# usnistgov/alignn

Hardware: NVIDIA B200
Metric: graphs/sec fwd+bwd (higher is better)
Workload: dtype f32

## Files before the change

### alignn_b200/_lib.py

```python
from __future__ import annotations

import ctypes as C
import os
from typing import Optional

import torch

_HERE = os.path.dirname(os.path.abspath(__file__))
LIB_PATH = os.path.join(_HERE, "libalignn_b200.so")

NORM_LAYER, NORM_AFFINE, NORM_STATS = 0, 1, 2
SUPPORTED_D = (32, 64, 128, 256)

_fp = C.c_void_p


class EgcFwdArgs(C.Structure):
    _fields_ = [
        ("struct_size", C.c_size_t),
        ("Nn", C.c_int64), ("Ne", C.c_int64),
        ("d", C.c_int32), ("norm_nodes", C.c_int32), ("norm_edges", C.c_int32), ("residual", C.c_int32),
        ("gate_is_m", C.c_int32),
        ("gate_eps", C.c_float), ("ln_eps", C.c_float),
        ("x", _fp), ("y", _fp), ("G", _fp), ("P", _fp),
        ("src", _fp), ("in_ptr", _fp), ("in_eid", _fp),
        ("n_w", _fp), ("n_b", _fp), ("e_w", _fp), ("e_b", _fp),
        ("x_out", _fp), ("y_out", _fp), ("M", _fp), ("XP", _fp), ("S", _fp), ("H", _fp),
        ("partials", _fp),
        ("stream", _fp),
    ]


class EgcBwdArgs(C.Structure):
    _fields_ = [
        ("struct_size", C.c_size_t),
        ("Nn", C.c_int64), ("Ne", C.c_int64),
        ("d", C.c_int32), ("norm_nodes", C.c_int32), ("norm_edges", C.c_int32),
        ("gate_eps", C.c_float), ("ln_eps", C.c_float),
        ("P", _fp), ("M", _fp), ("XP", _fp), ("S", _fp), ("H", _fp),
        ("src", _fp), ("dst", _fp), ("in_ptr", _fp), ("in_eid", _fp), ("out_ptr", _fp), ("out_eid", _fp),
        ("n_w", _fp), ("n_b", _fp), ("n_mean", _fp), ("n_rstd", _fp),
        ("e_w", _fp), ("e_b", _fp), ("e_mean", _fp), ("e_rstd", _fp),
        ("n_c1", _fp), ("n_c2", _fp), ("e_c1", _fp), ("e_c2", _fp),
        ("gx_out", _fp), ("gy_out", _fp),
        ("GM", _fp), ("GP", _fp), ("GSh", _fp),
        ("partials", _fp), ("partials_src", _fp),
        ("stream", _fp),
    ]


class GemmGatherArgs(C.Structure):
    _fields_ = [
        ("struct_size", C.c_size_t),
        ("M", C.c_int64), ("N", C.c_int32), ("K", C.c_int32),
        ("A", _fp), ("lda", C.c_int64),
        ("w_image", _fp), ("bias", _fp),
        ("add0", _fp), ("ld0", C.c_int64), ("idx0", _fp),
        ("add1", _fp), ("ld1", C.c_int64), ("idx1", _fp),
        ("C", _fp), ("ldc", C.c_int64),
        ("stats", _fp),
        ("bn_scale", _fp), ("bn_shift", _fp), ("bn_mean", _fp),
        ("stream", _fp),
    ]


class WgradProblem(C.Structure):
    _fields_ = [("A", _fp), ("lda", C.c_int64), ("B", _fp), ("ldb", C.c_int64), ("K", C.c_int64), ("out", _fp), ("ld_out", C.c_int64)]


class ColsumProblem(C.Structure):
    _fields_ = [("a", _fp), ("rows", C.c_int64), ("stride", C.c_int64), ("cols", C.c_int), ("alpha", C.c_float), ("out", _fp)]


class ImageEntry(C.Structure):
    _fields_ = [("W", _fp), ("ldw", C.c_int64), ("rows", C.c_int32), ("cols", C.c_int32), ("transpose", C.c_int32),
                ("n_off", C.c_int32), ("k_off", C.c_int32), ("N", C.c_int32), ("K", C.c_int32), ("image", _fp)]


class BiasEntry(C.Structure):
    _fields_ = [("a", _fp), ("b", _fp), ("dst", _fp), ("n", C.c_int32)]


_SIGNATURES = {
    "alignn_b200_version": (C.c_int, []),
    "alignn_b200_strerror": (C.c_char_p, [C.c_int]),
    "alignn_b200_last_cuda_error": (C.c_int, []),
    "alignn_b200_launch_count": (C.c_uint64, []),
    "alignn_b200_egc_partial_rows": (C.c_int, [C.c_int64, C.c_int]),
    "alignn_b200_egc_forward": (C.c_int, [C.POINTER(EgcFwdArgs)]),
    "alignn_b200_bn_finalize": (C.c_int, [_fp, C.c_int, C.c_int, C.c_int, C.c_int64, C.c_int, _fp, _fp, C.c_float,
                                          C.c_float, _fp, _fp, _fp, _fp, _fp, _fp, _fp]),
    "alignn_b200_affine_silu_residual": (C.c_int, [_fp, _fp, _fp, _fp, _fp, C.c_int64, C.c_int, _fp]),
    "alignn_b200_egc_backward": (C.c_int, [C.POINTER(EgcBwdArgs)]),
    "alignn_b200_bn_backward_reduce": (C.c_int, [_fp, _fp, _fp, _fp, _fp, _fp, C.c_int64, C.c_int, _fp, C.c_int, _fp]),
    "alignn_b200_rowstats_partials": (C.c_int, [_fp, C.c_int64, C.c_int, _fp, C.c_int, _fp]),
    "alignn_b200_bn_backward_apply": (C.c_int, [_fp, _fp, _fp, _fp, _fp, _fp, _fp, _fp, C.c_int64, C.c_int, _fp, _fp]),
    "alignn_b200_ln_silu_forward": (C.c_int, [_fp, _fp, _fp, C.c_float, C.c_int64, C.c_int, _fp, _fp, _fp]),
    "alignn_b200_ln_silu_backward": (C.c_int, [_fp, _fp, _fp, _fp, _fp, C.c_int64, C.c_int, _fp, _fp, C.c_int, _fp]),
    "alignn_b200_adamw_flat": (C.c_int, [_fp, _fp, _fp, _fp, C.c_int64, C.c_float, C.c_float, C.c_float, C.c_float, C.c_float,
                                         C.c_int, _fp, _fp, _fp]),
    "alignn_b200_colsum_partials": (C.c_int, [_fp, C.c_int64, C.c_int, _fp, C.c_int, _fp]),
    "alignn_b200_colsum": (C.c_int, [_fp, C.c_int64, C.c_int, C.c_int64, C.c_float, _fp, _fp]),
    "alignn_b200_colsum_batch": (C.c_int, [C.POINTER(ColsumProblem), C.c_int, _fp]),
    "alignn_b200_gather_segment_sum": (C.c_int, [_fp, _fp, _fp, _fp, _fp, C.c_int64, C.c_int64, C.c_int, _fp, _fp, _fp]),
    "alignn_b200_gemm_weight_image_bytes": (C.c_size_t, [C.c_int, C.c_int]),
    "alignn_b200_gemm_prepare_weights": (C.c_int, [_fp, C.c_int, C.c_int, C.c_int64, C.c_int, _fp, _fp]),
    "alignn_b200_gemm_prepare_table": (C.c_int, [_fp, C.c_int, C.c_int64, _fp, C.c_int, _fp]),
    "alignn_b200_gemm_nt": (C.c_int, [_fp, C.c_int64, _fp, C.c_int64, C.c_int, C.c_int, _fp, _fp, C.c_int64, _fp,
                                      C.c_int64, _fp]),
    "alignn_b200_gemm_gather": (C.c_int, [C.POINTER(GemmGatherArgs)]),
    "alignn_b200_gemm_gather_stat_rows": (C.c_int, [C.c_int64, C.c_int]),
    "alignn_b200_wgrad_workspace_bytes": (C.c_size_t, [C.c_int64, C.c_int, C.c_int, C.c_int]),
    "alignn_b200_wgrad_batch_workspace_bytes": (C.c_size_t, [C.POINTER(WgradProblem), C.c_int, C.c_int]),
    "alignn_b200_wgrad_batch": (C.c_int, [C.POINTER(WgradProblem), C.c_int, C.c_int, _fp, C.c_size_t, _fp]),
    "alignn_b200_wgrad": (C.c_int, [_fp, C.c_int64, _fp, C.c_int64, C.c_int64, C.c_int, C.c_int, C.c_int, _fp, C.c_int64,
                                    _fp, C.c_size_t, _fp]),
    "alignn_b200_csr_build_host": (C.c_int, [_fp, _fp, C.c_int64, C.c_int64, _fp, _fp, _fp, _fp, _fp, _fp, _fp, _fp]),
    "alignn_b200_line_graph_count_host": (C.c_int64, [_fp, _fp, _fp, C.c_int64]),
    "alignn_b200_line_graph_build_host": (C.c_int, [_fp, _fp, _fp, C.c_int64, _fp, C.c_int64, C.c_int64, _fp, _fp, _fp]),
    "alignn_b200_radius_graph_count_host": (C.c_int64, [_fp, _fp, C.c_int64, C.c_int64, C.c_double, C.c_double]),
    "alignn_b200_radius_graph_build_host": (C.c_int, [_fp, _fp, C.c_int64, C.c_int64, C.c_double, C.c_double, C.c_int64, _fp,
                                                      _fp, _fp, _fp]),
    "alignn_b200_csr_build_workspace_bytes": (C.c_size_t, [C.c_int64, C.c_int64]),
    "alignn_b200_csr_build": (C.c_int, [_fp, _fp, C.c_int64, C.c_int64, _fp, _fp, _fp, _fp, _fp, _fp, C.c_size_t, _fp]),
    "alignn_b200_line_graph_workspace_bytes": (C.c_size_t, [C.c_int64]),
    "alignn_b200_line_graph_offsets": (C.c_int, [_fp, _fp, _fp, C.c_int64, _fp, _fp, C.c_size_t, _fp]),
    "alignn_b200_line_graph_fill": (C.c_int, [_fp, _fp, _fp, _fp, C.c_int64, _fp, _fp, _fp, _fp]),
    "alignn_b200_radius_graph_workspace_bytes": (C.c_size_t, [C.c_int64]),
    "alignn_b200_radius_graph_offsets": (C.c_int, [_fp, _fp, C.c_int64, C.c_int64, C.c_double, C.c_double, _fp, _fp, C.c_size_t, _fp]),
    "alignn_b200_radius_graph_fill": (C.c_int, [_fp, _fp, C.c_int64, C.c_int64, C.c_double, C.c_double, _fp, _fp, _fp, _fp, _fp, _fp]),
    "alignn_b200_pair_force_scatter": (C.c_int, [_fp, _fp, _fp, _fp, _fp, C.c_int64, C.c_int, _fp, _fp]),
    "alignn_b200_virial_stress": (C.c_int, [_fp, _fp, _fp, _fp, _fp, C.c_int64, C.c_float, _fp, _fp]),
    "alignn_b200_debug_gemm_flags": (None, [C.c_int]),
    "alignn_b200_debug_gemm_pair": (None, [C.c_int]),
    "alignn_b200_debug_egc_flags": (None, [C.c_int]),
    "alignn_b200_debug_gemm_trace": (None, [_fp]),
    "alignn_b200_segment_mean": (C.c_int, [_fp, _fp, C.c_int64, C.c_int, _fp, _fp]),
    "alignn_b200_segment_mean_backward": (C.c_int, [_fp, _fp, C.c_int64, C.c_int, _fp, _fp]),
}

EXPORTED_SYMBOLS = tuple(_SIGNATURES)

_lib: Optional[C.CDLL] = None


def load() -> C.CDLL:
    global _lib
    if _lib is not None:
        return _lib
    if not os.path.exists(LIB_PATH):
        raise RuntimeError(
            f"{LIB_PATH} not found: the CUDA extension is not built. Run `python -c 'import __graft_entry__ as g; "
            "g.build()'` (nvcc, sm_100a). alignn_b200 has no CPU or eager fallback.")
    lib = C.CDLL(LIB_PATH)
    for name, (res, args) in _SIGNATURES.items():
        fn = getattr(lib, name)
        fn.restype, fn.argtypes = res, args
    if lib.alignn_b200_version() != 100:
        raise RuntimeError("libalignn_b200.so version mismatch; rebuild")
    _lib = lib
    return lib


def check(status: int, what: str) -> None:
    if status != 0:
        lib = load()
        msg = lib.alignn_b200_strerror(status).decode()
        extra = ""
        if status == -4:
            extra = f" (cudaError {lib.alignn_b200_last_cuda_error()})"
        raise RuntimeError(f"{what} failed: {msg}{extra}")


def launch_count() -> int:
    return int(load().alignn_b200_launch_count())


def ptr(t: Optional[torch.Tensor]):
    if t is None:
        return None
    return t.data_ptr()


def stream_ptr() -> int:
    return torch.cuda.current_stream().cuda_stream


def require_cuda(*tensors: torch.Tensor) -> None:
    for t in tensors:
        if t is None:
            continue
        if not t.is_cuda:
            raise RuntimeError("alignn_b200 kernels need CUDA tensors (no CPU path exists); got a tensor on "
                               f"{t.device}. Move the model and graphs to a B200 with .to('cuda').")
        if t.dtype not in (torch.float32, torch.int32):
            raise RuntimeError(f"alignn_b200 kernels are fp32/int32 only; got {t.dtype}")
        if not t.is_contiguous():
            raise RuntimeError("alignn_b200 kernels need contiguous tensors")
```

### alignn_b200/csrc/gemm_fused_tc.cu

```cuda
#include <atomic>
#include <cuda.h>

#include "tc_common.cuh"
#include "api_common.h"
#include "alignn_b200.h"

namespace alignn {
namespace gemm2 {

int make_map_f32(CUtensorMap* map, const float* base, int64_t rows, int64_t cols, int64_t ld, int box_rows);

constexpr int BM = 128;
constexpr int BK = 32;
constexpr int NSA = 3;
constexpr int NSP = 2;
constexpr int NSB = 3;
constexpr int EPI_WARPS = 8;
constexpr int CONV_WARPS = 4;
constexpr int THREADS = 32 * (4 + EPI_WARPS + CONV_WARPS);
constexpr uint32_t LBO = 128;
constexpr uint32_t SBO = (BK / 8) * 128;
constexpr int A_STAGE = BM * BK * 4;
constexpr int A_PLANE = BM * BK * 2;
constexpr int EPI_BOX = 32 * 32 * 4;
constexpr bool kTmaStore = true;
constexpr int EPI_BUFS = 1;

template <int BN>
struct Cfg {
  static constexpr int B_PLANE = BN * BK * 2;
  static constexpr int OFF_ASTG = 0;
  static constexpr int OFF_APL = OFF_ASTG + NSA * A_STAGE;
  static constexpr int OFF_B = OFF_APL + NSP * 2 * A_PLANE;
  static constexpr int OFF_EPI = (OFF_B + NSB * 2 * B_PLANE + 1023) / 1024 * 1024;
  static constexpr int EPI_BYTES = EPI_WARPS * EPI_BUFS * EPI_BOX;
  static constexpr int OFF_STAT = OFF_EPI + EPI_BYTES;
  static constexpr int STAT_BYTES = 4 * 2 * BN * 4;
  static constexpr int OFF_BAR = OFF_STAT + STAT_BYTES;
  static constexpr int SMEM = OFF_BAR + 256;
  static constexpr int TMEM_COLS = 2 * BN < 32 ? 32 : 2 * BN;
  static_assert(SMEM <= 232448, "shared memory budget of one sm_100 CTA");
};

struct Params {
  int M, N, K;
  const uint8_t* w_image;
  const float* bias;
  const float* add0; int64_t ld0; const int32_t* idx0;
  const float* add1; int64_t ld1; const int32_t* idx1;
  float* C; int64_t ldc;
  float* stats;
  int stat_quarters;
  const float* bn_scale; const float* bn_shift; const float* bn_mean;
  long long* trace;
};

#define GEMM2_TRACE(role, ctr) do { if (p.trace && blockIdx.x == 0 && (ctr) < 512) p.trace[(role) * 512 + (ctr)++] = clock64(); } while (0)

__host__ __device__ constexpr int plane_off(int r, int k) { return (r >> 3) * (int)SBO + (k >> 3) * 128 + (r & 7) * 16 + (k & 7) * 2; }

__device__ __forceinline__ float dsilu_(float u) {
  float e, sg;
  asm("ex2.approx.ftz.f32 %0, %1;" : "=f"(e) : "f"(u * -1.4426950408889634f));
  asm("rcp.approx.ftz.f32 %0, %1;" : "=f"(sg) : "f"(1.f + e));
  return sg * (1.f + u * (1.f - sg));
}
__device__ __forceinline__ void tma_load_2d(void* dst, const CUtensorMap* map, int c0, int c1, uint64_t* bar) {
  asm volatile("cp.async.bulk.tensor.2d.shared::cta.global.tile.mbarrier::complete_tx::bytes [%0], [%1, {%2, %3}], [%4];"
               ::"r"(tc::smem_u32(dst)), "l"(map), "r"(c0), "r"(c1), "r"(tc::smem_u32(bar)) : "memory");
}
__device__ __forceinline__ void tma_store_2d(const CUtensorMap* map, const void* src, int c0, int c1) {
  asm volatile("cp.async.bulk.tensor.2d.global.shared::cta.tile.bulk_group [%0, {%2, %3}], [%1];"
               ::"l"(map), "r"(tc::smem_u32(src)), "r"(c0), "r"(c1) : "memory");
}
__device__ __forceinline__ void tma_prefetch_2d(const CUtensorMap* map, int c0, int c1) {
  asm volatile("cp.async.bulk.prefetch.tensor.2d.L2.global.tile [%0, {%1, %2}];" ::"l"(map), "r"(c0), "r"(c1) : "memory");
}

template <int BN, int MODE>
__global__ void __launch_bounds__(THREADS, 1)
gemm_gather_bf16x3_kernel(const __grid_constant__ CUtensorMap mapA, const __grid_constant__ CUtensorMap mapC, const Params p) {
  using F = Cfg<BN>;
  extern __shared__ __align__(1024) uint8_t smem[];
  uint64_t* astg_full = reinterpret_cast<uint64_t*>(smem + F::OFF_BAR);
  uint64_t* astg_empty = astg_full + NSA;
  uint64_t* apl_full = astg_empty + NSA;
  uint64_t* apl_empty = apl_full + NSP;
  uint64_t* b_full = apl_empty + NSP;
  uint64_t* b_empty = b_full + NSB;
  uint64_t* tfull = b_empty + NSB;
  uint64_t* tempty = tfull + 2;
  uint32_t* tmem_slot = reinterpret_cast<uint32_t*>(tempty + 2);

  const int tid = threadIdx.x, warp = tid >> 5, lane = tid & 31;
  const int nk = p.K / BK;
  const int n_tiles = p.N / BN;
  const int m_tiles = (p.M + BM - 1) / BM;
  const int total = m_tiles * n_tiles;
  const int my_tiles = (total - (int)blockIdx.x + (int)gridDim.x - 1) / (int)gridDim.x;

  if (tid == 0) {
    for (int s = 0; s < NSA; ++s) { tc::mbar_init(&astg_full[s], 1); tc::mbar_init(&astg_empty[s], CONV_WARPS); }
    for (int s = 0; s < NSP; ++s) { tc::mbar_init(&apl_full[s], CONV_WARPS); tc::mbar_init(&apl_empty[s], 1); }
    for (int s = 0; s < NSB; ++s) { tc::mbar_init(&b_full[s], 1); tc::mbar_init(&b_empty[s], 1); }
    for (int a = 0; a < 2; ++a) { tc::mbar_init(&tfull[a], 1); tc::mbar_init(&tempty[a], EPI_WARPS); }
    tc::mbar_fence_init();
  }
  if (warp == 0) tc::tmem_alloc(tmem_slot, F::TMEM_COLS);
  tc::fence_before_sync();
  __syncthreads();
  tc::fence_after_sync();
  const uint32_t tmem = *tmem_slot;

  if (warp == 1) {
    if (lane == 0) {
      asm volatile("prefetch.tensormap [%0];" ::"l"(&mapA) : "memory");
      int c = 0, tr = 0;
      for (int lt = 0; lt < my_tiles; ++lt) {
        const int tile = blockIdx.x + lt * gridDim.x;
        const int m0 = (tile / n_tiles) * BM;
        if (lt + 1 < my_tiles) {
          const int nm0 = ((tile + (int)gridDim.x) / n_tiles) * BM;
          if (nm0 != m0)
            for (int kc = 0; kc < nk; ++kc) tma_prefetch_2d(&mapA, kc * BK, nm0);
        }
        for (int kc = 0; kc < nk; ++kc, ++c) {
          const int s = c % NSA;
          if (c >= NSA) tc::mbar_wait(&astg_empty[s], ((c / NSA) - 1) & 1);
          GEMM2_TRACE(0, tr);
          tc::mbar_arrive_expect_tx(&astg_full[s], A_STAGE);
          tma_load_2d(smem + F::OFF_ASTG + s * A_STAGE, &mapA, kc * BK, m0, &astg_full[s]);
        }
      }
    }
  } else if (warp == 2) {
    if (lane == 0) {
      int c = 0, trb = 0;
      for (int lt = 0; lt < my_tiles; ++lt) {
        const int tile = blockIdx.x + lt * gridDim.x;
        const uint8_t* wsrc = p.w_image + (int64_t)(tile % n_tiles) * nk * 2 * F::B_PLANE;
        for (int kc = 0; kc < nk; ++kc, ++c) {
          const int s = c % NSB;
          if (c >= NSB) tc::mbar_wait(&b_empty[s], ((c / NSB) - 1) & 1);
          GEMM2_TRACE(1, trb);
          tc::mbar_arrive_expect_tx(&b_full[s], 2 * F::B_PLANE);
          tc::bulk_g2s(smem + F::OFF_B + s * 2 * F::B_PLANE, wsrc, 2 * F::B_PLANE, &b_full[s]);
          wsrc += 2 * F::B_PLANE;
        }
      }
    }
  } else if (warp >= 4 + EPI_WARPS) {
    const int cw = warp - (4 + EPI_WARPS);
    int ld_off[8], st_off[8];
#pragma unroll
    for (int i = 0; i < 8; ++i) {
      const int u = (i * CONV_WARPS + cw) * 2 + (lane >> 4);
      const int row = (u >> 2) * 8 + (lane & 7);
      const int kq = (u & 3) * 2 + ((lane >> 3) & 1);
      ld_off[i] = row * 128 + ((kq ^ (row & 7)) << 4);
      st_off[i] = plane_off(row, kq * 4);
    }
    const int nchunks = my_tiles * nk;
    int tr2 = 0, tr3 = 0;
    for (int c = 0; c < nchunks; ++c) {
      const int sa = c % NSA, sp = c % NSP;
      tc::mbar_wait(&astg_full[sa], (c / NSA) & 1);
      if (cw == 0 && lane == 0) GEMM2_TRACE(2, tr2);
      const uint8_t* src = smem + F::OFF_ASTG + sa * A_STAGE;
      float4 v[8];
#pragma unroll
      for (int i = 0; i < 8; ++i) v[i] = *reinterpret_cast<const float4*>(src + ld_off[i]);
      if (c >= NSP) tc::mbar_wait(&apl_empty[sp], ((c / NSP) - 1) & 1);
      uint8_t* dst = smem + F::OFF_APL + sp * 2 * A_PLANE;
#pragma unroll
      for (int i = 0; i < 8; ++i) {
        uint2 hi, lo;
        tc::split4(v[i], hi, lo);
        *reinterpret_cast<uint2*>(dst + st_off[i]) = hi;
        *reinterpret_cast<uint2*>(dst + A_PLANE + st_off[i]) = lo;
      }
      tc::fence_async_smem();
      __syncwarp();
      if (lane == 0) {
        tc::mbar_arrive(&apl_full[sp]);
        tc::mbar_arrive(&astg_empty[sa]);
      }
      if (cw == 0 && lane == 0) GEMM2_TRACE(3, tr3);
    }
  } else if (warp >= 4) {
    const int ew = warp - 4;
    const int q = warp & 3;
    uint8_t* stg0 = smem + F::OFF_EPI + ew * EPI_BUFS * EPI_BOX;
    const int st_row = lane * 128, st_sw = lane & 7;
    uint32_t chunk_ctr = 0;
    float* stat = reinterpret_cast<float*>(smem + F::OFF_STAT) + q * 2 * BN;
    const int half = ew >> 2;
    constexpr bool bnmode = MODE == 1;
    constexpr bool plain = MODE == 2 && kTmaStore;
    constexpr bool one = MODE == 3;
    constexpr bool late_wait = (plain || one) && kTmaStore;
    const bool do_stats = !plain && !one && p.stats != nullptr;
    if (do_stats)
      for (int ch = half; ch < BN / 32; ch += 2) { stat[ch * 32 + lane] = 0.f; stat[BN + ch * 32 + lane] = 0.f; }
    const int rsub = lane >> 3;
    const int c4 = (lane & 7) * 4;
    constexpr int NCH = BN / 32;
    uint32_t lt = 0;
    int tr5 = 0;
    for (int tile = blockIdx.x; tile < total; tile += gridDim.x, ++lt) {
      const int acc = lt & 1;
      const int m0 = (tile / n_tiles) * BM, n0 = (tile % n_tiles) * BN;
      int i0[8], i1[8];
      uint32_t rvm = 0;
      const float* base0 = p.add0 + n0 + c4 + half * 32;
      const float* base1 = p.add1 + n0 + c4 + half * 32;
      float4 a0[8], a1[8];
      const float4 z4 = make_float4(0.f, 0.f, 0.f, 0.f);
      if constexpr (!plain) {
#pragma unroll
        for (int it = 0; it < 8; ++it) {
          const int gr = m0 + q * 32 + it * 4 + rsub;
          const bool ok = gr < p.M;
          rvm |= (ok ? 1u : 0u) << it;
          i0[it] = (p.add0 && ok) ? (p.idx0 ? __ldg(p.idx0 + gr) : gr) : -1;
          if constexpr (!one) i1[it] = (p.add1 && ok) ? (p.idx1 ? __ldg(p.idx1 + gr) : gr) : -1;
        }
#pragma unroll
        for (int it = 0; it < 8; ++it) {
          a0[it] = (i0[it] >= 0 && half < NCH) ? __ldg(reinterpret_cast<const float4*>(base0 + (int64_t)i0[it] * p.ld0)) : z4;
          if constexpr (!one)
            a1[it] = (i1[it] >= 0 && half < NCH) ? __ldg(reinterpret_cast<const float4*>(base1 + (int64_t)i1[it] * p.ld1)) : z4;
        }
      }
      tc::mbar_wait(&tfull[acc], (lt >> 1) & 1);
      tc::fence_after_sync();
      if (ew == 0 && lane == 0) GEMM2_TRACE(5, tr5);
#pragma unroll 1
      for (int ch = half; ch < NCH; ch += 2) {
        const int c0 = ch * 32;
        uint8_t* stg = stg0;
        if (!late_wait && kTmaStore && chunk_ctr >= 1) {
          if (lane == 0) asm volatile("cp.async.bulk.wait_group.read 0;" ::: "memory");
          __syncwarp();
        }
        {
          float v[32];
          tc::tmem_ld32(tmem + ((uint32_t)(q * 32) << 16) + (uint32_t)(acc * BN + c0), v);
          if (ew == 0 && lane == 0) GEMM2_TRACE(5, tr5);
          if (late_wait && chunk_ctr >= 1) {
            if (lane == 0) asm volatile("cp.async.bulk.wait_group.read 0;" ::: "memory");
            __syncwarp();
          }
          ++chunk_ctr;
          if constexpr (plain) {
            if (p.bias) {
#pragma unroll
              for (int j = 0; j < 8; ++j) {
                const float4 b = __ldg(reinterpret_cast<const float4*>(p.bias + n0 + c0 + 4 * j));
                v[4 * j] += b.x; v[4 * j + 1] += b.y; v[4 * j + 2] += b.z; v[4 * j + 3] += b.w;
              }
            }
          }
#pragma unroll
          for (int j = 0; j < 8; ++j)
            *reinterpret_cast<float4*>(stg + st_row + ((j ^ st_sw) << 4)) = make_float4(v[4 * j], v[4 * j + 1], v[4 * j + 2], v[4 * j + 3]);
        }
        if constexpr (plain) {
          tc::fence_async_smem();
          __syncwarp();
          if (ew == 0 && lane == 0) GEMM2_TRACE(5, tr5);
          if (lane == 0) {
            tma_store_2d(&mapC, stg, n0 + c0, m0 + q * 32);
            asm volatile("cp.async.bulk.commit_group;" ::: "memory");
          }
          __syncwarp();
          continue;
        }
        __syncwarp();
        if (ew == 0 && lane == 0) GEMM2_TRACE(5, tr5);
        float4 b4 = z4;
        if (p.bias) b4 = __ldg(reinterpret_cast<const float4*>(p.bias + n0 + c0 + c4));
        float4 bsc = z4, bsh = z4, bmu = z4;
        if (bnmode) {
          bsc = __ldg(reinterpret_cast<const float4*>(p.bn_scale + n0 + c0 + c4));
          bsh = __ldg(reinterpret_cast<const float4*>(p.bn_shift + n0 + c0 + c4));
          bmu = __ldg(reinterpret_cast<const float4*>(p.bn_mean + n0 + c0 + c4));
        }
        float4 s4 = z4, q4 = z4;
        const bool more = ch + 2 < NCH;
#pragma unroll
        for (int it = 0; it < 8; ++it) {
          const int r = it * 4 + rsub;
          float4* cell = reinterpret_cast<float4*>(stg + r * 128 + (((lane & 7) ^ (r & 7)) << 4));
          float4 o = *cell;
          float4 mrow = z4;
          if constexpr (!one) mrow = a1[it];
          const float4 ad1 = bnmode ? z4 : mrow;
          o.x = (o.x + b4.x) + (a0[it].x + ad1.x);
          o.y = (o.y + b4.y) + (a0[it].y + ad1.y);
          o.z = (o.z + b4.z) + (a0[it].z + ad1.z);
          o.w = (o.w + b4.w) + (a0[it].w + ad1.w);
          if (more) {
            if (i0[it] >= 0) a0[it] = __ldg(reinterpret_cast<const float4*>(base0 + (int64_t)i0[it] * p.ld0 + (c0 - half * 32) + 64));
            if constexpr (!one)
              if (i1[it] >= 0) a1[it] = __ldg(reinterpret_cast<const float4*>(base1 + (int64_t)i1[it] * p.ld1 + (c0 - half * 32) + 64));
          }
          if ((rvm >> it) & 1u) {
            if (bnmode) {
              float4 gu;
              gu.x = o.x * dsilu_(fmaf(mrow.x, bsc.x, bsh.x)); gu.y = o.y * dsilu_(fmaf(mrow.y, bsc.y, bsh.y));
              gu.z = o.z * dsilu_(fmaf(mrow.z, bsc.z, bsh.z)); gu.w = o.w * dsilu_(fmaf(mrow.w, bsc.w, bsh.w));
              s4.x += gu.x; s4.y += gu.y; s4.z += gu.z; s4.w += gu.w;
              q4.x = fmaf(gu.x, mrow.x - bmu.x, q4.x); q4.y = fmaf(gu.y, mrow.y - bmu.y, q4.y);
              q4.z = fmaf(gu.z, mrow.z - bmu.z, q4.z); q4.w = fmaf(gu.w, mrow.w - bmu.w, q4.w);
            } else {
              s4.x += o.x; s4.y += o.y; s4.z += o.z; s4.w += o.w;
              q4.x = fmaf(o.x, o.x, q4.x); q4.y = fmaf(o.y, o.y, q4.y); q4.z = fmaf(o.z, o.z, q4.z); q4.w = fmaf(o.w, o.w, q4.w);
            }
          }
          if constexpr (kTmaStore) *cell = o;
          else if ((rvm >> it) & 1u)
            *reinterpret_cast<float4*>(p.C + (int64_t)(m0 + q * 32 + r) * p.ldc + n0 + c0 + c4) = o;
        }
        if constexpr (kTmaStore) {
          tc::fence_async_smem();
          __syncwarp();
          if (lane == 0) {
            tma_store_2d(&mapC, stg, n0 + c0, m0 + q * 32);
            asm volatile("cp.async.bulk.commit_group;" ::: "memory");
          }
        } else {
          __syncwarp();
        }
        if (do_stats) {
#pragma unroll
          for (int o = 8; o <= 16; o <<= 1) {
            s4.x += __shfl_xor_sync(0xffffffffu, s4.x, o); s4.y += __shfl_xor_sync(0xffffffffu, s4.y, o);
            s4.z += __shfl_xor_sync(0xffffffffu, s4.z, o); s4.w += __shfl_xor_sync(0xffffffffu, s4.w, o);
            q4.x += __shfl_xor_sync(0xffffffffu, q4.x, o); q4.y += __shfl_xor_sync(0xffffffffu, q4.y, o);
            q4.z += __shfl_xor_sync(0xffffffffu, q4.z, o); q4.w += __shfl_xor_sync(0xffffffffu, q4.w, o);
          }
          if (lane < 8) {
            float4* ps = reinterpret_cast<float4*>(stat + c0 + c4);
            float4* pq = reinterpret_cast<float4*>(stat + BN + c0 + c4);
            float4 t = *ps; t.x += s4.x; t.y += s4.y; t.z += s4.z; t.w += s4.w; *ps = t;
            t = *pq; t.x += q4.x; t.y += q4.y; t.z += q4.z; t.w += q4.w; *pq = t;
          }
        }
        __syncwarp();
      }
      tc::fence_before_sync();
      __syncwarp();
      if (lane == 0) tc::mbar_arrive(&tempty[acc]);
      if (ew == 0 && lane == 0) GEMM2_TRACE(5, tr5);
    }
    if (kTmaStore && lane == 0) asm volatile("cp.async.bulk.wait_group 0;" ::: "memory");
    if (do_stats) {
      asm volatile("bar.sync 1, %0;" ::"n"(EPI_WARPS * 32) : "memory");
      const float* all = reinterpret_cast<const float*>(smem + F::OFF_STAT);
      if (p.stat_quarters == 4) {
        float* out_rows = p.stats + (int64_t)blockIdx.x * 4 * 2 * BN;
        for (int i = ew * 32 + lane; i < 4 * 2 * BN; i += EPI_WARPS * 32) out_rows[i] = all[i];
      } else {
        float* out_row = p.stats + (int64_t)blockIdx.x * 2 * BN;
        for (int i = ew * 32 + lane; i < 2 * BN; i += EPI_WARPS * 32)
          out_row[i] = (all[i] + all[2 * BN + i]) + (all[4 * BN + i] + all[6 * BN + i]);
      }
    }
  } else if (warp == 0 && lane == 0) {
    constexpr uint32_t IDESC = tc::idesc_bf16_f32(BM, BN);
    const uint64_t desc0 = tc::smem_desc(tc::smem_u32(smem), LBO, SBO);
    int c = 0, tr4 = 0;
    for (int lt = 0; lt < my_tiles; ++lt) {
      const int acc = lt & 1;
      if (lt >= 2) tc::mbar_wait(&tempty[acc], ((lt >> 1) - 1) & 1);
      tc::fence_after_sync();
      const uint32_t d_tmem = tmem + (uint32_t)(acc * BN);
      uint32_t accum = 0;
      for (int kc = 0; kc < nk; ++kc, ++c) {
        const int sp = c % NSP, sb = c % NSB;
        tc::mbar_wait(&apl_full[sp], (c / NSP) & 1);
        tc::mbar_wait(&b_full[sb], (c / NSB) & 1);
        tc::fence_after_sync();
        GEMM2_TRACE(4, tr4);
        const uint64_t da = desc0 + (uint64_t)((F::OFF_APL + sp * 2 * A_PLANE) >> 4);
        const uint64_t db = desc0 + (uint64_t)((F::OFF_B + sb * 2 * F::B_PLANE) >> 4);
#pragma unroll
        for (int j = 0; j < BK / 16; ++j) {
          const uint64_t a_hi = da + (uint64_t)((j * 2 * LBO) >> 4);
          const uint64_t a_lo = a_hi + (uint64_t)(A_PLANE >> 4);
          const uint64_t b_hi = db + (uint64_t)((j * 2 * LBO) >> 4);
          const uint64_t b_lo = b_hi + (uint64_t)(F::B_PLANE >> 4);
          tc::mma_bf16_ss(d_tmem, a_lo, b_hi, IDESC, accum);
          tc::mma_bf16_ss(d_tmem, a_hi, b_lo, IDESC, 1);
          tc::mma_bf16_ss(d_tmem, a_hi, b_hi, IDESC, 1);
          accum = 1;
        }
        tc::mma_commit(&apl_empty[sp]);
        tc::mma_commit(&b_empty[sb]);
      }
      tc::mma_commit(&tfull[acc]);
    }
  }
  tc::fence_before_sync();
  __syncthreads();
  if (warp == 0) tc::tmem_dealloc(tmem, F::TMEM_COLS);
}

typedef CUresult (*EncodeTiledFn)(CUtensorMap*, CUtensorMapDataType, cuuint32_t, void*, const cuuint64_t*, const cuuint64_t*,
                                  const cuuint32_t*, const cuuint32_t*, CUtensorMapInterleave, CUtensorMapSwizzle,
                                  CUtensorMapL2promotion, CUtensorMapFloatOOBfill);

static EncodeTiledFn encode_fn() {
  static std::atomic<EncodeTiledFn> cached{nullptr};
  EncodeTiledFn f = cached.load(std::memory_order_acquire);
  if (f) return f;
  void* sym = nullptr;
  cudaDriverEntryPointQueryResult q;
  if (cudaGetDriverEntryPoint("cuTensorMapEncodeTiled", &sym, cudaEnableDefault, &q) != cudaSuccess || !sym) return nullptr;
  f = reinterpret_cast<EncodeTiledFn>(sym);
  cached.store(f, std::memory_order_release);
  return f;
}

int make_map_f32(CUtensorMap* map, const float* base, int64_t rows, int64_t cols, int64_t ld, int box_rows) {
  EncodeTiledFn enc = encode_fn();
  if (!enc) return record_cuda_error((int)cudaErrorSymbolNotFound);
  cuuint64_t dims[2] = {(cuuint64_t)cols, (cuuint64_t)rows};
  cuuint64_t strides[1] = {(cuuint64_t)ld * 4};
  cuuint32_t box[2] = {32, (cuuint32_t)box_rows};
  cuuint32_t es[2] = {1, 1};
  CUresult r = enc(map, CU_TENSOR_MAP_DATA_TYPE_FLOAT32, 2, const_cast<float*>(base), dims, strides, box, es,
                   CU_TENSOR_MAP_INTERLEAVE_NONE, CU_TENSOR_MAP_SWIZZLE_128B, CU_TENSOR_MAP_L2_PROMOTION_L2_128B,
                   CU_TENSOR_MAP_FLOAT_OOB_FILL_NONE);
  if (r != CUDA_SUCCESS) return record_cuda_error(1000 + (int)r);
  return ALIGNN_OK;
}

static long long* g_trace = nullptr;

inline int pick_bn(int N) { return (N % 256 == 0) ? 256 : (N % 128 == 0) ? 128 : (N % 64 == 0) ? 64 : (N % 32 == 0) ? 32 : 0; }

template <int BN, int MODE>
int launch2(const CUtensorMap& mapA, const CUtensorMap& mapC, const Params& p, cudaStream_t st) {
  using F = Cfg<BN>;
  static alignn::DeviceOnce configured; int cfg_dev;
  if (configured.needed(&cfg_dev)) {
    cudaError_t e = cudaFuncSetAttribute(gemm_gather_bf16x3_kernel<BN, MODE>, cudaFuncAttributeMaxDynamicSharedMemorySize, F::SMEM);
    if (e != cudaSuccess) return record_cuda_error((int)e);
    configured.done(cfg_dev);
  }
  const int total = ((p.M + BM - 1) / BM) * (p.N / BN);
  int grid = total < 148 ? total : 148;
  if (p.stats) grid = alignn_b200_gemm_gather_stat_rows(p.M, p.N) / p.stat_quarters;
  gemm_gather_bf16x3_kernel<BN, MODE><<<grid, THREADS, F::SMEM, st>>>(mapA, mapC, p);
  return check_launch();
}

template <int BN>
int launch(const CUtensorMap& mapA, const CUtensorMap& mapC, const Params& p, cudaStream_t st) {
  if (p.bn_scale) return launch2<BN, 1>(mapA, mapC, p, st);
  if (kTmaStore && !p.add0 && !p.add1 && !p.stats) return launch2<BN, 2>(mapA, mapC, p, st);
  if (p.add0 && !p.add1 && !p.stats) return launch2<BN, 3>(mapA, mapC, p, st);
  return launch2<BN, 0>(mapA, mapC, p, st);
}

}
}

extern "C" {

void alignn_b200_debug_gemm_trace(long long* device_buffer) { alignn::gemm2::g_trace = device_buffer; }

__attribute__((visibility("hidden"))) int alignn_b200_gemm_pair_enabled();

int alignn_b200_gemm_gather_stat_rows(int64_t M, int N) {
  const int bn = alignn::gemm2::pick_bn(N);
  if (bn == 0 || M <= 0) return 0;
  const int64_t total = 2 * ((M + 2 * alignn::gemm2::BM - 1) / (2 * alignn::gemm2::BM));
  return (alignn_b200_gemm_pair_enabled() ? 4 : 1) * (int)(total < 148 ? total : 148);
}

__attribute__((visibility("hidden"))) int alignn_b200_gemm_gather_try_pair(const alignn_b200_gemm_gather_args* a, int* status);

int alignn_b200_gemm_gather(const alignn_b200_gemm_gather_args* a) {
  using namespace alignn::gemm2;
  if (!a) return ALIGNN_ERR_BAD_ARG;
  if (a->struct_size != sizeof(*a)) return ALIGNN_ERR_STRUCT_SIZE;
  if (a->M < 0 || a->N <= 0 || a->K <= 0 || a->K % BK != 0 || a->lda < a->K || a->ldc < a->N) return ALIGNN_ERR_BAD_ARG;
  if (a->M == 0) return ALIGNN_OK;
  if (!a->A || !a->w_image || !a->C || a->M > 0x7fffffff) return ALIGNN_ERR_BAD_ARG;
  if ((a->lda % 4) || (a->ldc % 4) || ((uintptr_t)a->A & 15) || ((uintptr_t)a->C & 15)) return ALIGNN_ERR_BAD_ARG;
  if (a->add0 && ((a->ld0 % 4) || a->ld0 < a->N || ((uintptr_t)a->add0 & 15))) return ALIGNN_ERR_BAD_ARG;
  if (a->add1 && ((a->ld1 % 4) || a->ld1 < a->N || ((uintptr_t)a->add1 & 15))) return ALIGNN_ERR_BAD_ARG;
  if ((a->idx0 && !a->add0) || (a->idx1 && !a->add1)) return ALIGNN_ERR_BAD_ARG;
  const int bn = pick_bn(a->N);
  if (bn == 0) return ALIGNN_ERR_UNSUPPORTED_D;
  if (a->stats && a->N != bn) return ALIGNN_ERR_BAD_ARG;
  if (a->bn_scale && (!a->bn_shift || !a->bn_mean || !a->add1 || !a->stats)) return ALIGNN_ERR_BAD_ARG;
  {
    int st = ALIGNN_OK;
    if (alignn_b200_gemm_gather_try_pair(a, &st)) return st;
  }
  CUtensorMap mapA, mapC;
  int rc = make_map_f32(&mapA, a->A, a->M, a->K, a->lda, BM);
  if (rc != ALIGNN_OK) return rc;
  rc = make_map_f32(&mapC, a->C, a->M, a->N, a->ldc, 32);
  if (rc != ALIGNN_OK) return rc;
  Params p;
  p.M = (int)a->M; p.N = a->N; p.K = a->K;
  p.w_image = reinterpret_cast<const uint8_t*>(a->w_image);
  p.bias = a->bias;
  p.add0 = a->add0; p.ld0 = a->ld0; p.idx0 = a->idx0;
  p.add1 = a->add1; p.ld1 = a->ld1; p.idx1 = a->idx1;
  p.C = a->C; p.ldc = a->ldc; p.stats = a->stats; p.stat_quarters = alignn_b200_gemm_pair_enabled() ? 4 : 1;
  p.bn_scale = a->bn_scale; p.bn_shift = a->bn_shift; p.bn_mean = a->bn_mean;
  p.trace = g_trace;
  cudaStream_t st = (cudaStream_t)a->stream;
  switch (bn) {
    case 256: return launch<256>(mapA, mapC, p, st);
    case 128: return launch<128>(mapA, mapC, p, st);
    case 64: return launch<64>(mapA, mapC, p, st);
    default: return launch<32>(mapA, mapC, p, st);
  }
}

}
```

### include/alignn_b200.h

```cpp
#ifndef ALIGNN_B200_H
#define ALIGNN_B200_H

#include <stddef.h>
#include <stdint.h>

#ifdef __cplusplus
extern "C" {
#endif

#define ALIGNN_B200_VERSION 100

typedef enum {
  ALIGNN_OK = 0,
  ALIGNN_ERR_BAD_ARG = -1,
  ALIGNN_ERR_UNSUPPORTED_D = -2,
  ALIGNN_ERR_STRUCT_SIZE = -3,
  ALIGNN_ERR_CUDA = -4,
  ALIGNN_ERR_WORKSPACE = -5
} alignn_b200_status;

typedef enum {
  ALIGNN_NORM_LAYER = 0,
  ALIGNN_NORM_AFFINE = 1,
  ALIGNN_NORM_STATS = 2
} alignn_b200_norm;

typedef void* alignn_stream_t;

int alignn_b200_version(void);
const char* alignn_b200_strerror(int status);
int alignn_b200_last_cuda_error(void);
uint64_t alignn_b200_launch_count(void);

int alignn_b200_egc_partial_rows(int64_t Nn, int d);

typedef struct {
  size_t struct_size;
  int64_t Nn, Ne;
  int32_t d;
  int32_t norm_nodes, norm_edges;
  int32_t residual;
  int32_t gate_is_m;
  float gate_eps;
  float ln_eps;
  const float* x;
  const float* y;
  const float* G;
  const float* P;
  const int32_t* src;
  const int32_t* in_ptr;
  const int32_t* in_eid;
  const float* n_w; const float* n_b;
  const float* e_w; const float* e_b;
  float* x_out;
  float* y_out;
  float* M;
  float* XP;
  float* S;
  float* H;
  float* partials;
  alignn_stream_t stream;
} alignn_b200_egc_fwd_args;

int alignn_b200_egc_forward(const alignn_b200_egc_fwd_args* args);

int alignn_b200_bn_finalize(const float* partials, int partial_rows, int partial_stride ,
                            int which ,
                            int64_t count, int d, const float* gamma, const float* beta, float eps, float momentum,
                            float* running_mean, float* running_var ,
                            float* scale, float* shift, float* mean, float* rstd, alignn_stream_t stream);

int alignn_b200_affine_silu_residual(const float* R, const float* res, const float* scale, const float* shift,
                                     float* out, int64_t n, int d, alignn_stream_t stream);

typedef struct {
  size_t struct_size;
  int64_t Nn, Ne;
  int32_t d;
  int32_t norm_nodes, norm_edges;
  float gate_eps, ln_eps;
  const float* P; const float* M; const float* XP; const float* S; const float* H;
  const int32_t* src; const int32_t* dst;
  const int32_t* in_ptr; const int32_t* in_eid;
  const int32_t* out_ptr; const int32_t* out_eid;
  const float* n_w; const float* n_b; const float* n_mean; const float* n_rstd;
  const float* e_w; const float* e_b; const float* e_mean; const float* e_rstd;
  const float* n_c1; const float* n_c2; const float* e_c1; const float* e_c2;
  const float* gx_out;
  const float* gy_out;
  float* GM; float* GP;
  float* GSh;
  float* partials;
  float* partials_src;
  alignn_stream_t stream;
} alignn_b200_egc_bwd_args;

int alignn_b200_egc_backward(const alignn_b200_egc_bwd_args* args);

int alignn_b200_bn_backward_reduce(const float* R, const float* g_out, const float* scale, const float* shift,
                                   const float* mean, const float* rstd, int64_t n, int d,
                                   float* partials, int partial_rows, alignn_stream_t stream);

int alignn_b200_rowstats_partials(const float* a, int64_t n, int d, float* partials, int partial_rows, alignn_stream_t stream);
int alignn_b200_bn_backward_apply(const float* R, const float* g_out, const float* scale, const float* shift,
                                  const float* mean, const float* rstd, const float* c1, const float* c2, int64_t n, int d,
                                  float* gR, alignn_stream_t stream);

int alignn_b200_ln_silu_forward(const float* h, const float* gamma, const float* beta, float eps, int64_t n, int d, float* out,
                                float* rowstat, alignn_stream_t stream);
int alignn_b200_ln_silu_backward(const float* h, const float* g_out, const float* rowstat, const float* gamma, const float* beta,
                                 int64_t n, int d, float* gh, float* partials, int partial_rows, alignn_stream_t stream);

int alignn_b200_adamw_flat(float* param, float* grad, float* exp_avg, float* exp_avg_sq, int64_t n, float lr, float beta1,
                           float beta2, float eps, float weight_decay, int zero_grad, int64_t* step, uint32_t* ticket,
                           alignn_stream_t stream);

int alignn_b200_colsum_partials(const float* a, int64_t n, int d, float* partials, int partial_rows, alignn_stream_t stream);

int alignn_b200_colsum(const float* a, int64_t rows, int cols, int64_t stride, float alpha, float* out,
                       alignn_stream_t stream);

typedef struct {
  const float* a; int64_t rows; int64_t stride;
  int cols; float alpha;
  float* out;
} alignn_b200_colsum_problem;
int alignn_b200_colsum_batch(const alignn_b200_colsum_problem* problems, int n, alignn_stream_t stream);

int alignn_b200_gather_segment_sum(const float* Bh, const float* sigma, const int32_t* src,
                                   const int32_t* in_ptr, const int32_t* in_eid, int64_t Nn, int64_t Ne, int d,
                                   float* Sh, float* S, alignn_stream_t stream);

size_t alignn_b200_gemm_weight_image_bytes(int N, int K);
int alignn_b200_gemm_prepare_weights(const float* W, int N, int K, int64_t ldw, int transpose, void* image,
                                     alignn_stream_t stream);
typedef struct {
  const float* W; int64_t ldw;
  int32_t rows, cols, transpose;
  int32_t n_off, k_off;
  int32_t N, K;
  void* image;
} alignn_b200_image_entry;
typedef struct { const float* a; const float* b; float* dst; int32_t n; } alignn_b200_bias_entry;
int alignn_b200_gemm_prepare_table(const alignn_b200_image_entry* entries, int n_entries, int64_t max_units,
                                   const alignn_b200_bias_entry* bias_entries, int n_bias, alignn_stream_t stream);
int alignn_b200_gemm_nt(const float* A, int64_t lda, const void* w_image, int64_t M, int N, int K, const float* bias,
                        const float* R, int64_t ldr, float* C, int64_t ldc, alignn_stream_t stream);

typedef struct {
  size_t struct_size;
  int64_t M; int32_t N, K;
  const float* A; int64_t lda;
  const void* w_image;
  const float* bias;
  const float* add0; int64_t ld0; const int32_t* idx0;
  const float* add1; int64_t ld1; const int32_t* idx1;
  float* C; int64_t ldc;
  float* stats;
  const float* bn_scale; const float* bn_shift; const float* bn_mean;
  alignn_stream_t stream;
} alignn_b200_gemm_gather_args;

int alignn_b200_gemm_gather(const alignn_b200_gemm_gather_args* args);
int alignn_b200_gemm_gather_stat_rows(int64_t M, int N);

size_t alignn_b200_wgrad_workspace_bytes(int64_t K, int DA, int DB, int groups);
int alignn_b200_wgrad(const float* A, int64_t lda, const float* B, int64_t ldb, int64_t K, int DA, int DB, int groups,
                      float* out, int64_t ld_out, void* workspace, size_t workspace_bytes, alignn_stream_t stream);

typedef struct {
  const float* A; int64_t lda;
  const float* B; int64_t ldb;
  int64_t K;
  float* out; int64_t ld_out;
} alignn_b200_wgrad_problem;
size_t alignn_b200_wgrad_batch_workspace_bytes(const alignn_b200_wgrad_problem* problems, int n, int D);
int alignn_b200_wgrad_batch(const alignn_b200_wgrad_problem* problems, int n, int D, void* workspace, size_t workspace_bytes,
                            alignn_stream_t stream);

int alignn_b200_csr_build_host(const int64_t* src, const int64_t* dst, int64_t num_nodes, int64_t num_edges,
                               int32_t* src32, int32_t* dst32, int32_t* in_ptr, int32_t* in_eid, int32_t* out_ptr,
                               int32_t* out_eid, int32_t* dst_sorted, int32_t* max_in_degree);
int64_t alignn_b200_line_graph_count_host(const int32_t* src, const int32_t* in_ptr, const int32_t* in_eid,
                                          int64_t num_edges);
int alignn_b200_line_graph_build_host(const int32_t* src, const int32_t* in_ptr, const int32_t* in_eid,
                                      int64_t num_edges, const int64_t* batch_num_edges, int64_t batch_size,
                                      int64_t capacity, int64_t* lsrc, int64_t* ldst, int64_t* l_batch_num_edges);

int64_t alignn_b200_radius_graph_count_host(const double* cart_coords, const double* shifts, int64_t num_atoms,
                                            int64_t num_images, double cutoff, double atol);
int alignn_b200_radius_graph_build_host(const double* cart_coords, const double* shifts, int64_t num_atoms,
                                        int64_t num_images, double cutoff, double atol, int64_t capacity, int64_t* u,
                                        int64_t* v, int64_t* image_index, float* r);

size_t alignn_b200_csr_build_workspace_bytes(int64_t num_nodes, int64_t num_edges);
int alignn_b200_csr_build(const int32_t* src, const int32_t* dst, int64_t num_nodes, int64_t num_edges, int32_t* in_ptr,
                          int32_t* in_eid, int32_t* out_ptr, int32_t* out_eid, int32_t* flags, void* workspace,
                          size_t workspace_bytes, alignn_stream_t stream);

size_t alignn_b200_line_graph_workspace_bytes(int64_t num_edges);
int alignn_b200_line_graph_offsets(const int32_t* src, const int32_t* dst, const int32_t* in_ptr, int64_t num_edges,
                                   int32_t* offsets, void* workspace, size_t workspace_bytes, alignn_stream_t stream);
int alignn_b200_line_graph_fill(const int32_t* src, const int32_t* dst, const int32_t* in_ptr, const int32_t* in_eid,
                                int64_t num_edges, const int32_t* offsets, int32_t* lsrc, int32_t* ldst, alignn_stream_t stream);

size_t alignn_b200_radius_graph_workspace_bytes(int64_t num_atoms);
int alignn_b200_radius_graph_offsets(const double* cart_coords, const double* shifts, int64_t num_atoms, int64_t num_images,
                                     double cutoff, double atol, int32_t* offsets, void* workspace, size_t workspace_bytes,
                                     alignn_stream_t stream);
int alignn_b200_radius_graph_fill(const double* cart_coords, const double* shifts, int64_t num_atoms, int64_t num_images,
                                  double cutoff, double atol, const int32_t* offsets, int32_t* u, int32_t* v,
                                  int32_t* image_index, float* r, alignn_stream_t stream);

int alignn_b200_pair_force_scatter(const float* pair_forces, const int32_t* in_ptr, const int32_t* in_eid,
                                   const int32_t* out_ptr, const int32_t* out_eid, int64_t num_nodes, int add_reverse,
                                   float* forces, alignn_stream_t stream);

int alignn_b200_virial_stress(const float* r, const float* pair_forces, const int64_t* edge_offsets,
                              const int64_t* node_offsets, const float* V, int64_t batch_size, float multiplier,
                              float* stress, alignn_stream_t stream);

int alignn_b200_segment_mean(const float* x, const int32_t* graph_ptr , int64_t B, int d, float* out,
                             alignn_stream_t stream);
int alignn_b200_segment_mean_backward(const float* g_out , const int32_t* graph_ptr, int64_t B, int d,
                                      float* gx , alignn_stream_t stream);

void alignn_b200_debug_gemm_flags(int flags);
void alignn_b200_debug_gemm_pair(int enabled);
void alignn_b200_debug_egc_flags(int flags);
void alignn_b200_debug_gemm_trace(long long* device_buffer);

#ifdef __cplusplus
}
#endif
#endif
```

Measured before the change: 8263.

## Pick narrower GEMM N-tile via cost model to fill SMs on small launches

Adds a per-launch cost model that picks a narrower N tile (half or quarter of the weight-image block width) when the number of M×N tiles is small, so more CTAs run across the 148 SMs. The weight loader now slices sub-blocks out of the wider pre-packed image using two bulk copies, and the stats epilogue writes per-column-range partial rows with zero-fill for unused rows. This trades higher per-tile overhead and repeated A loads for better SM occupancy. Cost-model constants are hardcoded fits, and the pair mode keeps the old width.

```diff
diff --git a/alignn_b200/_lib.py b/alignn_b200/_lib.py
--- a/alignn_b200/_lib.py
+++ b/alignn_b200/_lib.py
@@ -110,6 +110,7 @@
                                       C.c_int64, _fp]),
     "alignn_b200_gemm_gather": (C.c_int, [C.POINTER(GemmGatherArgs)]),
     "alignn_b200_gemm_gather_stat_rows": (C.c_int, [C.c_int64, C.c_int]),
+    "alignn_b200_gemm_gather_tile_n": (C.c_int, [C.c_int64, C.c_int, C.c_int, C.c_int]),
     "alignn_b200_wgrad_workspace_bytes": (C.c_size_t, [C.c_int64, C.c_int, C.c_int, C.c_int]),
     "alignn_b200_wgrad_batch_workspace_bytes": (C.c_size_t, [C.POINTER(WgradProblem), C.c_int, C.c_int]),
     "alignn_b200_wgrad_batch": (C.c_int, [C.POINTER(WgradProblem), C.c_int, C.c_int, _fp, C.c_size_t, _fp]),
@@ -133,6 +134,7 @@
     "alignn_b200_virial_stress": (C.c_int, [_fp, _fp, _fp, _fp, _fp, C.c_int64, C.c_float, _fp, _fp]),
     "alignn_b200_debug_gemm_flags": (None, [C.c_int]),
     "alignn_b200_debug_gemm_pair": (None, [C.c_int]),
+    "alignn_b200_debug_gemm_tile_n": (None, [C.c_int]),
     "alignn_b200_debug_egc_flags": (None, [C.c_int]),
     "alignn_b200_debug_gemm_trace": (None, [_fp]),
     "alignn_b200_segment_mean": (C.c_int, [_fp, _fp, C.c_int64, C.c_int, _fp, _fp]),
diff --git a/alignn_b200/csrc/gemm_fused_tc.cu b/alignn_b200/csrc/gemm_fused_tc.cu
--- a/alignn_b200/csrc/gemm_fused_tc.cu
+++ b/alignn_b200/csrc/gemm_fused_tc.cu
@@ -45,11 +45,13 @@
 struct Params {
   int M, N, K;
   const uint8_t* w_image;
+  int bi;
   const float* bias;
   const float* add0; int64_t ld0; const int32_t* idx0;
   const float* add1; int64_t ld1; const int32_t* idx1;
   float* C; int64_t ldc;
   float* stats;
+  int stat_rows;
   int stat_quarters;
   const float* bn_scale; const float* bn_shift; const float* bn_mean;
   long long* trace;
@@ -135,17 +137,26 @@
     }
   } else if (warp == 2) {
     if (lane == 0) {
+      const int64_t chunk_bytes = (int64_t)p.bi * BK * 2 * 2;
+      const int64_t plane_bytes = chunk_bytes / 2;
       int c = 0, trb = 0;
       for (int lt = 0; lt < my_tiles; ++lt) {
         const int tile = blockIdx.x + lt * gridDim.x;
-        const uint8_t* wsrc = p.w_image + (int64_t)(tile % n_tiles) * nk * 2 * F::B_PLANE;
+        const int n0 = (tile % n_tiles) * BN;
+        const uint8_t* wsrc = p.w_image + (int64_t)(n0 / p.bi) * nk * chunk_bytes + (int64_t)(n0 % p.bi) * BK * 2;
         for (int kc = 0; kc < nk; ++kc, ++c) {
           const int s = c % NSB;
           if (c >= NSB) tc::mbar_wait(&b_empty[s], ((c / NSB) - 1) & 1);
           GEMM2_TRACE(1, trb);
           tc::mbar_arrive_expect_tx(&b_full[s], 2 * F::B_PLANE);
-          tc::bulk_g2s(smem + F::OFF_B + s * 2 * F::B_PLANE, wsrc, 2 * F::B_PLANE, &b_full[s]);
-          wsrc += 2 * F::B_PLANE;
+          uint8_t* dst = smem + F::OFF_B + s * 2 * F::B_PLANE;
+          if (p.bi == BN) {
+            tc::bulk_g2s(dst, wsrc, 2 * F::B_PLANE, &b_full[s]);
+          } else {
+            tc::bulk_g2s(dst, wsrc, F::B_PLANE, &b_full[s]);
+            tc::bulk_g2s(dst + F::B_PLANE, wsrc + plane_bytes, F::B_PLANE, &b_full[s]);
+          }
+          wsrc += chunk_bytes;
         }
       }
     }
@@ -362,9 +373,14 @@
         float* out_rows = p.stats + (int64_t)blockIdx.x * 4 * 2 * BN;
         for (int i = ew * 32 + lane; i < 4 * 2 * BN; i += EPI_WARPS * 32) out_rows[i] = all[i];
       } else {
-        float* out_row = p.stats + (int64_t)blockIdx.x * 2 * BN;
+        const int own_rows = (int)gridDim.x / n_tiles;
+        const int n0 = ((int)blockIdx.x % n_tiles) * BN;
+        float* out_row = p.stats + (int64_t)((int)blockIdx.x / n_tiles) * 2 * p.N + n0;
         for (int i = ew * 32 + lane; i < 2 * BN; i += EPI_WARPS * 32)
-          out_row[i] = (all[i] + all[2 * BN + i]) + (all[4 * BN + i] + all[6 * BN + i]);
+          out_row[(i / BN) * p.N + i % BN] = (all[i] + all[2 * BN + i]) + (all[4 * BN + i] + all[6 * BN + i]);
+        for (int r = own_rows + (int)blockIdx.x / n_tiles; r < p.stat_rows; r += own_rows)
+          for (int i = ew * 32 + lane; i < 2 * BN; i += EPI_WARPS * 32)
+            p.stats[(int64_t)r * 2 * p.N + (i / BN) * p.N + n0 + i % BN] = 0.f;
       }
     }
   } else if (warp == 0 && lane == 0) {
@@ -450,20 +466,49 @@
     if (e != cudaSuccess) return record_cuda_error((int)e);
     configured.done(cfg_dev);
   }
-  const int total = ((p.M + BM - 1) / BM) * (p.N / BN);
+  const int n_tiles = p.N / BN;
+  const int total = ((p.M + BM - 1) / BM) * n_tiles;
   int grid = total < 148 ? total : 148;
-  if (p.stats) grid = alignn_b200_gemm_gather_stat_rows(p.M, p.N) / p.stat_quarters;
+  if (p.stats) {
+    if (n_tiles == 1) grid = p.stat_rows / p.stat_quarters;
+    else grid -= grid % n_tiles;
+  }
   gemm_gather_bf16x3_kernel<BN, MODE><<<grid, THREADS, F::SMEM, st>>>(mapA, mapC, p);
   return check_launch();
 }
 
 template <int BN>
-int launch(const CUtensorMap& mapA, const CUtensorMap& mapC, const Params& p, cudaStream_t st) {
-  if (p.bn_scale) return launch2<BN, 1>(mapA, mapC, p, st);
-  if (kTmaStore && !p.add0 && !p.add1 && !p.stats) return launch2<BN, 2>(mapA, mapC, p, st);
-  if (p.add0 && !p.add1 && !p.stats) return launch2<BN, 3>(mapA, mapC, p, st);
-  return launch2<BN, 0>(mapA, mapC, p, st);
-}
+int launch(const CUtensorMap& mapA, const CUtensorMap& mapC, const Params& p, cudaStream_t st, int mode) {
+  switch (mode) {
+    case 1: return launch2<BN, 1>(mapA, mapC, p, st);
+    case 2: return launch2<BN, 2>(mapA, mapC, p, st);
+    case 3: return launch2<BN, 3>(mapA, mapC, p, st);
+    default: return launch2<BN, 0>(mapA, mapC, p, st);
+  }
+}
+
+inline int mode_of(const alignn_b200_gemm_gather_args* a) {
+  if (a->bn_scale) return 1;
+  if (kTmaStore && !a->add0 && !a->add1 && !a->stats) return 2;
+  if (a->add0 && !a->add1 && !a->stats) return 3;
+  return 0;
+}
+
+struct TileCost { double fixed, per_k, per_col; };
+inline const TileCost& tile_cost(int mode) {
+  static const TileCost row_pass2 = {-1.71, 0.0184, 0.0365};
+  static const TileCost row_pass1 = {-1.45, 0.0184, 0.0243};
+  static const TileCost plain = {-0.90, 0.0184, 0.0133};
+  return mode == 2 ? plain : mode == 3 ? row_pass1 : row_pass2;
+}
+
+inline double launch_cost(int64_t M, int K, int N, int bn, int mode) {
+  const TileCost& c = tile_cost(mode);
+  const int64_t tiles = ((M + BM - 1) / BM) * (N / bn);
+  return (double)((tiles + 147) / 148) * (c.fixed + c.per_k * K + c.per_col * bn);
+}
+
+static std::atomic<int> g_tile_n{0};
 
 }
 }
@@ -473,6 +518,23 @@
 void alignn_b200_debug_gemm_trace(long long* device_buffer) { alignn::gemm2::g_trace = device_buffer; }
 
 __attribute__((visibility("hidden"))) int alignn_b200_gemm_pair_enabled();
+
+void alignn_b200_debug_gemm_tile_n(int bn) { alignn::gemm2::g_tile_n.store(bn); }
+
+int alignn_b200_gemm_gather_tile_n(int64_t M, int N, int K, int mode) {
+  using namespace alignn::gemm2;
+  const int bi = pick_bn(N);
+  if (bi == 0 || M <= 0 || K <= 0 || mode < 0 || mode > 3) return 0;
+  if (((M + BM - 1) / BM) * (N / bi) > 5 * 148)
+    return ((mode == 0 || mode == 3) && K >= 256 && bi >= 128) ? bi / 2 : bi;
+  int best = bi;
+  double best_cost = launch_cost(M, K, N, bi, mode);
+  for (int bn = bi / 2; bn >= 64 && bn >= bi / 4; bn /= 2) {
+    const double c = launch_cost(M, K, N, bn, mode);
+    if (c < best_cost) { best = bn; best_cost = c; }
+  }
+  return best;
+}
 
 int alignn_b200_gemm_gather_stat_rows(int64_t M, int N) {
   const int bn = alignn::gemm2::pick_bn(N);
@@ -513,16 +575,23 @@
   p.bias = a->bias;
   p.add0 = a->add0; p.ld0 = a->ld0; p.idx0 = a->idx0;
   p.add1 = a->add1; p.ld1 = a->ld1; p.idx1 = a->idx1;
-  p.C = a->C; p.ldc = a->ldc; p.stats = a->stats; p.stat_quarters = alignn_b200_gemm_pair_enabled() ? 4 : 1;
+  const bool pair = alignn_b200_gemm_pair_enabled();
+  p.C = a->C; p.ldc = a->ldc; p.stats = a->stats; p.stat_quarters = pair ? 4 : 1;
+  p.stat_rows = a->stats ? alignn_b200_gemm_gather_stat_rows(a->M, a->N) : 0;
   p.bn_scale = a->bn_scale; p.bn_shift = a->bn_shift; p.bn_mean = a->bn_mean;
   p.trace = g_trace;
+  p.bi = bn;
+  const int mode = mode_of(a);
+  int tn = pair ? bn : alignn_b200_gemm_gather_tile_n(a->M, a->N, a->K, mode);
+  const int forced = g_tile_n.load();
+  if (forced != 0 && !pair) tn = (forced >= 64 && forced <= bn && bn % forced == 0) ? forced : bn;
   cudaStream_t st = (cudaStream_t)a->stream;
-  switch (bn) {
-    case 256: return launch<256>(mapA, mapC, p, st);
-    case 128: return launch<128>(mapA, mapC, p, st);
-    case 64: return launch<64>(mapA, mapC, p, st);
-    default: return launch<32>(mapA, mapC, p, st);
-  }
-}
-
-}
+  switch (tn) {
+    case 256: return launch<256>(mapA, mapC, p, st, mode);
+    case 128: return launch<128>(mapA, mapC, p, st, mode);
+    case 64: return launch<64>(mapA, mapC, p, st, mode);
+    default: return launch<32>(mapA, mapC, p, st, mode);
+  }
+}
+
+}
diff --git a/include/alignn_b200.h b/include/alignn_b200.h
--- a/include/alignn_b200.h
+++ b/include/alignn_b200.h
@@ -163,6 +163,7 @@
 
 int alignn_b200_gemm_gather(const alignn_b200_gemm_gather_args* args);
 int alignn_b200_gemm_gather_stat_rows(int64_t M, int N);
+int alignn_b200_gemm_gather_tile_n(int64_t M, int N, int K, int mode);
 
 size_t alignn_b200_wgrad_workspace_bytes(int64_t K, int DA, int DB, int groups);
 int alignn_b200_wgrad(const float* A, int64_t lda, const float* B, int64_t ldb, int64_t K, int DA, int DB, int groups,
@@ -227,6 +228,7 @@
 
 void alignn_b200_debug_gemm_flags(int flags);
 void alignn_b200_debug_gemm_pair(int enabled);
+void alignn_b200_debug_gemm_tile_n(int bn);
 void alignn_b200_debug_egc_flags(int flags);
 void alignn_b200_debug_gemm_trace(long long* device_buffer);
 
```

Result: faster. 8456, median of 6 (+2.3%).
